# ppwwyyxx/OpenPano

Measured on NVIDIA H100. Metric: Mpixels/sec SIFT+match+blend, higher is better.
Workload: dtype f32

## Files before the change

openpano_b200/capi.py:

```python
from __future__ import annotations

import ctypes as C
import os
from pathlib import Path

import numpy as np

from ._abi import (PanoBaLink, PanoBaPair, PanoBlendGeom, PanoCylJob, PanoBlendImage, PanoMatches, PanoParams, PanoRansacPair, PanoSSPoint,
                   default_params)

LIB_PATH = Path(__file__).resolve().parent / "libpano_b200.so"

_fp = C.POINTER(C.c_float)
_dp = C.POINTER(C.c_double)
_ip = C.POINTER(C.c_int)
_vpp = C.POINTER(C.c_void_p)

SSPOINT_DTYPE = np.dtype([("x", "<i4"), ("y", "<i4"), ("real_x", "<f8"), ("real_y", "<f8"),
                          ("pyr_id", "<i4"), ("scale_id", "<i4"), ("dir", "<f4"),
                          ("scale_factor", "<f4")], align=True)


class PanoError(RuntimeError):
    def __init__(self, code, msg):
# ... 302 lines not shown
    def profile(self, on: bool):
        self._check(LIB.pano_profile_enable(self._h, 1 if on else 0))

    def profile_reset(self):
        self._check(LIB.pano_profile_reset(self._h))

    def profile_read(self):
        cap = 64
        names = C.create_string_buffer(cap * 64)
        launches = (C.c_int * cap)()
        ms = (C.c_double * cap)()
        n = LIB.pano_profile_read(self._h, cap, names, launches, ms)
        out = {}
        for i in range(min(n, cap)):
            nm = names.raw[i * 64:(i + 1) * 64].split(b"\0", 1)[0].decode()
            out[nm] = (launches[i], ms[i])
        return out

    def dev_alloc(self, nbytes):
        p = C.c_void_p()
        self._check(LIB.pano_dev_alloc(self._h, nbytes, C.byref(p)))
        return p.value

    def dev_free(self, ptr):
        LIB.pano_dev_free(self._h, C.c_void_p(ptr))

    def dev_upload(self, ptr, arr):
        arr = np.ascontiguousarray(arr)
        self._check(LIB.pano_dev_upload(self._h, C.c_void_p(ptr), arr.ctypes.data_as(C.c_void_p), arr.nbytes))

    def dev_download(self, arr, ptr):
        assert arr.flags.c_contiguous
        self._check(LIB.pano_dev_download(self._h, arr.ctypes.data_as(C.c_void_p), C.c_void_p(ptr), arr.nbytes))

    def dev_upload_async(self, d_ptr, h_ptr, nbytes):
        self._check(LIB.pano_dev_upload_async(self._h, C.c_void_p(d_ptr), C.c_void_p(h_ptr), nbytes))

    def dev_download_async(self, h_ptr, d_ptr, nbytes):
        self._check(LIB.pano_dev_download_async(self._h, C.c_void_p(h_ptr), C.c_void_p(d_ptr), nbytes))

    @staticmethod
    def host_alloc(nbytes):
        p = C.c_void_p()
        if LIB.pano_host_alloc(nbytes, C.byref(p)) != 0:
            raise PanoError(-1, "pano_host_alloc failed")
        return p.value

    @staticmethod
    def host_free(ptr):
        LIB.pano_host_free(C.c_void_p(ptr))

    def event_create(self):
        e = C.c_void_p()
        self._check(LIB.pano_event_create(self._h, C.byref(e)))
        return e

    def event_record(self, ev):
        self._check(LIB.pano_event_record(self._h, ev))

    def event_wait(self, ev):
        self._check(LIB.pano_event_wait(self._h, ev))

    @staticmethod
    def event_sync(ev):
        if LIB.pano_event_sync(ev) != 0:
            raise PanoError(-1, "pano_event_sync failed")

    @staticmethod
    def event_destroy(ev):
        LIB.pano_event_destroy(ev)

    def sift_detect_batch(self, imgs, params=None) -> FeatureSet:
        params = params or default_params()
        imgs = [np.ascontiguousarray(im, np.float32) for im in imgs]
        n = len(imgs)
        ptrs = (C.c_void_p * n)(*[im.ctypes.data for im in imgs])
        ws = (C.c_int * n)(*[im.shape[1] for im in imgs])
        hs = (C.c_int * n)(*[im.shape[0] for im in imgs])
        out = C.c_void_p()
        self._check(LIB.pano_sift_detect_batch(self._h, n, ptrs, ws, hs, C.byref(params), C.byref(out)))
        return FeatureSet(self, out)

    def sift_detect_batch_ptr(self, ptrs, ws, hs, params=None, device=False) -> FeatureSet:
        params = params or default_params()
        n = len(ptrs)
        cp = (C.c_void_p * n)(*ptrs)
        cw = (C.c_int * n)(*ws)
        ch = (C.c_int * n)(*hs)
        out = C.c_void_p()
        fn = LIB.pano_sift_detect_batch_dev if device else LIB.pano_sift_detect_batch
        self._check(fn(self._h, n, cp, cw, ch, C.byref(params), C.byref(out)))
        return FeatureSet(self, out)

    def sift_detect(self, img, params=None):
        fs = self.sift_detect_batch([img], params)
        try:
            return fs.download(0)
        finally:
            fs.free()

    def sift_trace(self, img, params=None) -> GpuSiftTrace:
        params = params or default_params()
        img = np.ascontiguousarray(img, np.float32)
        out = C.c_void_p()
        self._check(LIB.pano_sift_trace_run(self._h, _f(img), img.shape[1], img.shape[0], C.byref(params),
                                            C.byref(out)))
        return GpuSiftTrace(self, out)

    def featureset_upload(self, descs, coors=None) -> FeatureSet:
        descs = [np.ascontiguousarray(d, np.float32).reshape(-1, 128) for d in descs]
        n = len(descs)
        cnt = (C.c_int * n)(*[len(d) for d in descs])
        dp = (C.c_void_p * n)(*[d.ctypes.data for d in descs])
        cp = None
        if coors is not None:
            coors = [np.ascontiguousarray(c, np.float64).reshape(-1, 2) for c in coors]
            cp = (C.c_void_p * n)(*[c.ctypes.data for c in coors])
        out = C.c_void_p()
        self._check(LIB.pano_featureset_upload(self._h, n, cnt, dp, cp, C.byref(out)))
        return FeatureSet(self, out)

    def featureset_import_dev(self, counts, d_descs, d_coors=None) -> FeatureSet:
        n = len(counts)
        cnt = (C.c_int * n)(*counts)
        dp = (C.c_void_p * n)(*d_descs)
        cp = (C.c_void_p * n)(*d_coors) if d_coors is not None else None
        out = C.c_void_p()
        self._check(LIB.pano_featureset_import_dev(self._h, n, cnt, dp, cp, C.byref(out)))
        return FeatureSet(self, out)

    def blend_rows_dev(self, ptrs, shapes, items, geom, d_out_rows, out_w, out_h, row0, row1, bands=0, params=None):
        params = params or default_params()
        arr, g = self._blend_args(ptrs, shapes, items, geom)
        self._check(LIB.pano_blend_rows_dev(self._h, len(ptrs), arr, C.byref(g), bands, C.byref(params),
                                            C.c_void_p(d_out_rows), out_w, out_h, row0, row1))

    def match_pairs(self, fs: FeatureSet, pairs, params=None, shard=(0, 1)):
        params = params or default_params()
        pairs = np.ascontiguousarray(pairs, np.int32).reshape(-1, 2)
        m = PanoMatches()
        self._check(LIB.pano_match_pairs_shard(self._h, fs._h, len(pairs), _i(pairs), C.byref(params), int(shard[0]),
                                               int(shard[1]), C.byref(m)))
        n = m.n_pairs
        offs = np.ctypeslib.as_array(m.offset, shape=(n + 1,)).copy() if n else np.zeros(1, np.int32)
        total = int(offs[n]) if n else 0
        idx = (np.ctypeslib.as_array(m.idx, shape=(2 * total,)).reshape(-1, 2).copy() if total
               else np.zeros((0, 2), np.int32))
        LIB.pano_matches_free(C.byref(m))
        return [idx[offs[k]:offs[k + 1]] for k in range(n)]

    def match_pairs_dev(self, fs: FeatureSet, pairs, params=None, shard=(0, 1)) -> int:
        params = params or default_params()
        pairs = np.ascontiguousarray(pairs, np.int32).reshape(-1, 2)
        tot = C.c_int()
        self._check(LIB.pano_match_pairs_dev_shard(self._h, fs._h, len(pairs), _i(pairs), C.byref(params), int(shard[0]),
                                                   int(shard[1]), C.byref(tot)))
        return tot.value

    def match_bruteforce(self, a, b, params=None):
        params = params or default_params()
        a = np.ascontiguousarray(a, np.float32).reshape(-1, 128)
        b = np.ascontiguousarray(b, np.float32).reshape(-1, 128)
        pairs = np.zeros((max(1, min(len(a), len(b))), 2), np.int32)
        n = C.c_int()
        self._check(LIB.pano_match_bruteforce(self._h, _f(a), len(a), _f(b), len(b), C.byref(params),
                                              _i(pairs), C.byref(n)))
        return pairs[:n.value].copy()

    def ransac_score_pairs(self, pairs):
        n = len(pairs)
        arr = (PanoRansacPair * max(n, 1))()
# ... 22 lines not shown
            C.memmove(arr[k].m, np.ascontiguousarray(mats, np.float64).ctypes.data, 13 * 9 * 8)
            begin += nm
        pts_to = np.ascontiguousarray(pts_to, np.float64).reshape(-1, 2)
        assert len(pts_to) == begin
        rows = np.zeros((max(begin, 1), 24), np.float64) if want_rows else None
        jtj = np.full((6 * n_cam, 6 * n_cam), np.nan, np.float64)
        self._check(LIB.pano_ba_jacobian(self._h, n_cam, n, arr, _d(pts_to), _d(rows) if want_rows else None, _d(jtj)))
        return (rows[:begin] if want_rows else None), jtj

    def ba_session(self, n_cam, pairs, pts) -> BaSession:
        n = len(pairs)
        arr = (PanoBaLink * max(n, 1))()
        begin = 0
        for k, (f, t, nm) in enumerate(pairs):
            arr[k].from_, arr[k].to, arr[k].match_begin, arr[k].n_match = f, t, begin, nm
            begin += nm
        pts = np.ascontiguousarray(pts, np.float64).reshape(-1, 4)
        if len(pts) != begin:
            raise PanoError(-2, f"ba session: {len(pts)} coordinate rows for {begin} matches")
        h = C.c_void_p()
        self._check(LIB.pano_ba_session_create(self._h, n_cam, n, arr, _d(pts) if len(pts) else None, C.byref(h)))
        return BaSession(self, h, n_cam, n, begin)

    @staticmethod
    def cyl_warp_shape(w, h, h_factor=1.0, params=None):
        params = params or default_params()
        ow, oh, ox, oy = C.c_int(), C.c_int(), C.c_double(), C.c_double()
        rc = LIB.pano_cyl_warp_shape(w, h, h_factor, C.byref(params), C.byref(ow), C.byref(oh), C.byref(ox),
                                     C.byref(oy))
        if rc:
            raise PanoError(rc, "pano_cyl_warp_shape")
        return ow.value, oh.value, ox.value, oy.value

    def cyl_warp(self, img, kpts=None, h_factor=1.0, params=None):
        params = params or default_params()
        img = np.ascontiguousarray(img, np.float32)
        ow, oh, _, _ = self.cyl_warp_shape(img.shape[1], img.shape[0], h_factor, params)
        out = np.empty((oh, ow, 3), np.float32)
        k = np.ascontiguousarray(kpts if kpts is not None else np.zeros((0, 2)), np.float64).copy()
        self._check(LIB.pano_cyl_warp(self._h, _f(img), img.shape[1], img.shape[0], h_factor, C.byref(params),
                                      _f(out), ow, oh, _d(k), len(k)))
        return out, k

    def cyl_warp_batch_dev(self, src_ptrs, shapes, dst_ptrs, kpts=None, h_factor=1.0, params=None):
        params = params or default_params()
        n = len(src_ptrs)
        arr = (PanoCylJob * max(n, 1))()
        for k in range(n):
            h, w = shapes[k]
            ow, oh, _, _ = self.cyl_warp_shape(w, h, h_factor, params)
            arr[k].d_rgb_hwc, arr[k].w, arr[k].h = src_ptrs[k], w, h
            arr[k].d_out_hwc, arr[k].out_w, arr[k].out_h = dst_ptrs[k], ow, oh
            if kpts is not None and kpts[k] is not None and len(kpts[k]):
                assert kpts[k].dtype == np.float64 and kpts[k].flags["C_CONTIGUOUS"]
                arr[k].kpts_xy, arr[k].n_kpts = kpts[k].ctypes.data, len(kpts[k])
        self._check(LIB.pano_cyl_warp_batch_dev(self._h, n, arr, h_factor, C.byref(params)))

    @staticmethod
    def _blend_args(imgs_or_ptrs, shapes, items, geom):
        n = len(items)
        arr = (PanoBlendImage * n)()
        for k in range(n):
            arr[k].rgb_hwc = imgs_or_ptrs[k]
            arr[k].h, arr[k].w = shapes[k]
            arr[k].x0, arr[k].y0, arr[k].x1, arr[k].y1 = items[k][:4]
            for q in range(9):
                arr[k].homo_inv[q] = items[k][4][q]
        g = PanoBlendGeom(projection=geom["projection"], res_x=geom["res_x"], res_y=geom["res_y"],
                          proj_min_x=geom["proj_min_x"], proj_min_y=geom["proj_min_y"])
        return arr, g

    def blend(self, imgs, items, geom, bands=0, params=None):
        params = params or default_params()
        imgs = [np.ascontiguousarray(im, np.float32) for im in imgs]
        arr, g = self._blend_args([im.ctypes.data for im in imgs], [im.shape[:2] for im in imgs], items, geom)
        ow, oh = C.c_int(), C.c_int()
        LIB.pano_blend_target_size(len(imgs), arr, C.byref(ow), C.byref(oh))
        out = np.empty((oh.value, ow.value, 3), np.float32)
        self._check(LIB.pano_blend(self._h, len(imgs), arr, C.byref(g), bands, C.byref(params), _f(out),
                                   ow.value, oh.value))
        return out

    def blend_dev(self, ptrs, shapes, items, geom, d_out, out_w, out_h, bands=0, params=None):
        params = params or default_params()
        arr, g = self._blend_args(ptrs, shapes, items, geom)
        self._check(LIB.pano_blend_dev(self._h, len(ptrs), arr, C.byref(g), bands, C.byref(params),
                                       C.c_void_p(d_out), out_w, out_h))

    PLANET_SIZE = 1000

    def planet(self, img):
        img = np.ascontiguousarray(img, np.float32)
        if img.ndim != 3 or img.shape[2] != 3:
            raise PanoError(-2, f"planet: expected an H×W×3 image, got shape {img.shape}")
        out = np.empty((self.PLANET_SIZE, self.PLANET_SIZE, 3), np.float32)
        self._check(LIB.pano_planet(self._h, _f(img), img.shape[1], img.shape[0], _f(out)))
        return out

    def planet_dev(self, d_src, w, h, d_out):
        self._check(LIB.pano_planet_dev(self._h, C.c_void_p(d_src or 0), w, h, C.c_void_p(d_out or 0)))

    def rgb8_to_mat32f_batch_dev(self, d_pix, ws, hs, channels, d_out):
        n = len(d_pix)
        src = (C.c_void_p * n)(*d_pix)
        dst = (C.c_void_p * n)(*d_out)
        self._check(LIB.pano_rgb8_to_mat32f_batch_dev(self._h, n, src, (C.c_int * n)(*ws), (C.c_int * n)(*hs),
                                                      (C.c_int * n)(*channels), dst))

    def rgb8_to_mat32f_dev(self, d_pix, w, h, channels, d_out):
        self._check(LIB.pano_rgb8_to_mat32f_dev(self._h, C.c_void_p(d_pix), w, h, channels, C.c_void_p(d_out)))

    def crop_rect_dev(self, d_mat, w, h, d_rect):
        self._check(LIB.pano_crop_rect_dev(self._h, C.c_void_p(d_mat), w, h, C.c_void_p(d_rect)))

    def mat32f_to_rgb8_dev(self, d_mat, w, h, d_rect, d_out):
        self._check(LIB.pano_mat32f_to_rgb8_dev(self._h, C.c_void_p(d_mat), w, h, C.c_void_p(d_rect or 0),
                                                C.c_void_p(d_out)))

    def read_img_rgb8(self, pix):
        pix = np.ascontiguousarray(pix, np.uint8)
        h, w = pix.shape[:2]
        ch = 1 if pix.ndim == 2 else pix.shape[2]
        d_in = self.dev_alloc(max(pix.nbytes, 256))
        d_out = self.dev_alloc(h * w * 12)
        out = np.empty((h, w, 3), np.float32)
        try:
            self.dev_upload(d_in, pix)
            self.rgb8_to_mat32f_dev(d_in, w, h, ch, d_out)
            self.dev_download(out, d_out)
        finally:
            self.dev_free(d_in)
            self.dev_free(d_out)
        return out

    def crop_write_rgb8(self, mat, crop=True):
        mat = np.ascontiguousarray(mat, np.float32)
        h, w = mat.shape[:2]
        d_mat = self.dev_alloc(mat.nbytes)
        d_rect = self.dev_alloc(256)
        d_out = self.dev_alloc(max(h * w * 3, 256))
        rect = np.zeros(4, np.int32)
        out = np.empty(h * w * 3, np.uint8)
        try:
            self.dev_upload(d_mat, mat)
            if crop:
                self.crop_rect_dev(d_mat, w, h, d_rect)
            self.mat32f_to_rgb8_dev(d_mat, w, h, d_rect if crop else 0, d_out)
            self.dev_download(out, d_out)
            if crop:
                self.dev_download(rect, d_rect)
        finally:
            for p_ in (d_mat, d_rect, d_out):
                self.dev_free(p_)
        if not crop:
            return None, out.reshape(h, w, 3)
        cw, ch = int(rect[2]), int(rect[3])
        return rect, out[:cw * ch * 3].reshape(ch, cw, 3).copy()
```

openpano_b200/csrc/match.cu:

```cuda
#include "sift.cuh"
#include "match_tc.cuh"
#include <float.h>
#include <stdlib.h>
#include <string.h>
#include <algorithm>

__device__ __forceinline__ float exact_dist(const float* __restrict__ a, const float* __restrict__ b) {
  float l0 = 0.f, l1 = 0.f, l2 = 0.f, l3 = 0.f;
  const float4* pa = (const float4*)a;
  const float4* pb = (const float4*)b;
#pragma unroll 8
  for (int k = 0; k < 32; ++k) {
    float4 x = __ldg(pa + k), y = __ldg(pb + k);
    float d0 = x.x - y.x, d1 = x.y - y.y, d2 = x.z - y.z, d3 = x.w - y.w;
    l0 += d0 * d0; l1 += d1 * d1; l2 += d2 * d2; l3 += d3 * d3;
  }
  return (l0 + l1) + (l2 + l3);
}

__device__ __forceinline__ void top2_merge(float& mn, int& idx, float& sec, float m2, int i2, float s2) {
  if (m2 < mn || (m2 == mn && i2 < idx)) { sec = fminf(mn, s2); mn = m2; idx = i2; }
  else sec = fminf(sec, m2);
}

// ... 632 lines not shown
                (long long)pl.res_total, rs, pl.lazy ? 1 : 0, b.info);
  }
  if (pl.max_small > 0) {
    int block_cap = (int)std::min<size_t>(std::max<size_t>(pl.tc_tasks.size(), 1), 4096);
    if (const char* e = getenv("PANO_MATCH_BLOCK_CAP")) block_cap = std::max(1, std::min(block_cap, atoi(e)));
    const size_t grow = (size_t)block_cap * 128;
    TcFilter f;
    if ((rc = ctx_alloc(ctx, (void**)&b.list_rows, nres * sizeof(int))) ||
        (rc = ctx_alloc(ctx, (void**)&b.gtasks, (size_t)block_cap * sizeof(TcTask))) ||
        (rc = ctx_alloc(ctx, (void**)&b.gq, (size_t)block_cap * tc_block_bytes())) ||
        (rc = ctx_alloc(ctx, (void**)&b.g_meta, grow * sizeof(int2))) ||
        (rc = ctx_alloc(ctx, (void**)&b.g_thr, grow * sizeof(int))) ||
        (rc = ctx_alloc(ctx, (void**)&b.cand_cnt, grow * sizeof(int))) ||
        (rc = ctx_alloc(ctx, (void**)&b.cand, grow * TC_CAND_CAP * sizeof(int))))
      return rc;
    f.gq = b.gq; f.tasks = b.gtasks; f.gsides = b.gsides; f.list_rows = b.list_rows; f.approx = b.approx;
    f.g_meta = b.g_meta; f.g_thr = b.g_thr; f.cand_cnt = b.cand_cnt; f.cand = b.cand;
    TcFilter nf;
    int nom_cap = 0;
    if (pl.lazy) {
      nom_cap = (int)std::min<long long>(std::max<long long>(pl.large_blocks, 1), 8192);
      const size_t nrow = (size_t)nom_cap * 128;
      if ((rc = ctx_alloc(ctx, (void**)&b.list_unknown, nres * sizeof(int))) ||
          (rc = ctx_alloc(ctx, (void**)&b.ntasks, (size_t)nom_cap * sizeof(TcTask))) ||
          (rc = ctx_alloc(ctx, (void**)&b.nq, (size_t)nom_cap * tc_block_bytes())) ||
          (rc = ctx_alloc(ctx, (void**)&b.n_meta, nrow * sizeof(int2))) ||
          (rc = ctx_alloc(ctx, (void**)&b.n_approx, nrow * sizeof(TcTop2))))
        return rc;
      nf.gq = b.nq; nf.tasks = b.ntasks; nf.gsides = b.gsides; nf.list_rows = b.list_unknown; nf.approx = nullptr;
      nf.g_meta = b.n_meta; nf.g_thr = nullptr; nf.cand_cnt = nullptr; nf.cand = nullptr;
    }
    int* list_unknown = pl.lazy ? b.list_unknown : b.list_rows;
    const int eg = ctx->num_sms * 4;
    b.rounds = pl.lazy ? 3 : 2;
    for (int round = 0; round <= b.rounds; ++round) {
      int* side_cnt = b.counters + MC_HEAD + round * 2 * n_sides;
      int* fb_cnt = b.counters + MC_FB(round);
      int* n_blocks = b.counters + MC_BLK_FILTER(round);
      PANO_LAUNCH(ctx, "k_match_decide", k_match_decide, gd, 256, 0, b.pairs, b.sides, b.info, rs, round == 0 ? 1 : 0,
                  b.out, b.counters, b.list_rows, list_unknown, side_cnt, n_sides);
      if (round == b.rounds) break;
      if (pl.lazy) {
        int* nom_blocks = b.counters + MC_BLK_NOMINATE(round);
        PANO_LAUNCH(ctx, "k_gather_plan", k_gather_plan, ceil_div(n_sides, 128), 128, 0, b.gsides, n_sides,
                    side_cnt + n_sides, b.list_unknown, nom_cap, b.ntasks, nom_blocks, b.list, fb_cnt);
        nf.n_tasks = nom_blocks;
        if ((rc = tc_run_nominate(ctx, ops, &nf, nom_cap, b.n_approx))) return rc;
        PANO_LAUNCH(ctx, "k_refine_gathered", k_refine_gathered, nom_cap, 128, 0, fs->d_desc, ops->d_norms, ops->d_maxnorm,
                    b.sides, b.n_meta, b.n_approx, nom_blocks, rs, b.approx, b.info);
      }
      PANO_LAUNCH(ctx, "k_gather_plan", k_gather_plan, ceil_div(n_sides, 128), 128, 0, b.gsides, n_sides, side_cnt,
                  b.list_rows, block_cap, b.gtasks, n_blocks, b.list, fb_cnt);
      f.n_tasks = n_blocks;
      if ((rc = tc_run_filter(ctx, ops, &f, block_cap))) return rc;
      PANO_LAUNCH(ctx, "k_exact_cands", k_exact_cands, eg, 256, 0, fs->d_desc, b.sides, n_blocks, b.g_meta, b.cand_cnt,
                  b.cand, b.info, b.list, fb_cnt);
      PANO_LAUNCH(ctx, "k_exact_rows", k_exact_rows, eg, 256, 0, fs->d_desc, b.sides, b.list, fb_cnt, b.info);
    }
  }
  return PANO_OK;
}

static int ensure_tc_operands(pano_ctx* ctx, pano_featureset* fs, std::vector<TcImage>& imgs) {
  imgs.resize(fs->n_images);
  int blk = 0;
  for (int i = 0; i < fs->n_images; ++i) {
    TcImage& im = imgs[i];
    im.row0 = fs->base[i]; im.n = fs->h_count[i];
    im.n_pad = (im.n + 255) / 256 * 256;
    im.blk0 = blk;
    blk += im.n_pad / 128;
  }
  if (fs->tc_ready) return PANO_OK;
  int rc = tc_prepare(ctx, fs->d_desc, imgs, &fs->tc);
  if (rc) return rc;
  fs->tc_ready = true;
  return PANO_OK;
}

static int match_common(pano_ctx* ctx, pano_featureset* fs, int n_pairs, const int* ij, const pano_params* p,
                        int shard, int n_shards, MatchPlan& pl, MatchBuffers& b) {
  if (n_shards < 1 || shard < 0 || shard >= n_shards) return ctx_fail(ctx, PANO_ERR_INVALID, "shard %d of %d", shard, n_shards);
  pl.shard = shard; pl.n_shards = n_shards;
  int rc = featureset_sync_counts(fs);
  if (rc) return rc;
  const bool tensor = !use_exact_path();
  std::vector<TcImage> tcimgs;
  if (tensor && (rc = ensure_tc_operands(ctx, fs, tcimgs))) return rc;
  rc = build_plan(ctx, fs, n_pairs, ij, pl, tensor ? &tcimgs : nullptr);
  if (rc) return rc;
  return run_plan(ctx, fs, pl, p->match_reject_next_ratio, tensor, &fs->tc, b);
}

extern "C" {

int pano_match_pairs(pano_ctx* ctx, pano_featureset* fs, int n_pairs, const int* ij, const pano_params* p,
                     pano_matches* out) {
  return pano_match_pairs_shard(ctx, fs, n_pairs, ij, p, 0, 1, out);
}

int pano_match_pairs_shard(pano_ctx* ctx, pano_featureset* fs, int n_pairs, const int* ij, const pano_params* p,
                           int shard, int n_shards, pano_matches* out) {
  ctx_enter(ctx);
  if (!ctx || !fs || !out || n_pairs < 0 || (n_pairs && !ij) || !p) return PANO_ERR_INVALID;
  memset(out, 0, sizeof(*out));
  MatchPlan pl;
  MatchBuffers b;
  int rc = match_common(ctx, fs, n_pairs, ij, p, shard, n_shards, pl, b);
  if (rc) { free_buffers(ctx, b, false); return rc; }
  const size_t n_hdr = 3 + 2 * (size_t)n_pairs;
  const size_t cap = (size_t)std::max<long long>(pl.out_total, 1) * 2;
  int *d_hdr = nullptr, *d_dense = nullptr;
  if ((rc = ctx_alloc(ctx, (void**)&d_hdr, n_hdr * sizeof(int))) || (rc = ctx_alloc(ctx, (void**)&d_dense, cap * sizeof(int)))) {
    ctx_free(ctx, d_hdr); ctx_free(ctx, d_dense); free_buffers(ctx, b, false); return rc;
  }
  int* h_stage = (int*)ctx_ring(ctx, (n_hdr + cap) * sizeof(int));
  if (!h_stage) { ctx_free(ctx, d_hdr); ctx_free(ctx, d_dense); free_buffers(ctx, b, false); return ctx_fail(ctx, PANO_ERR_CUDA, "pinned ring allocation failed"); }
  auto finish = [&](int code) { ctx_free(ctx, d_hdr); ctx_free(ctx, d_dense); free_buffers(ctx, b, false); return code; };
  if ((rc = ctx_zero(ctx, d_hdr, 2 * sizeof(int)))) return finish(rc);
  if (n_pairs > 0) {
    ctx->launches += 4;
    k_match_count<<<n_pairs, 256, 0, ctx->stream>>>(b.pairs, b.out, n_pairs, d_hdr);
    k_match_offsets<<<1, 1024, 0, ctx->stream>>>(n_pairs, d_hdr);
    k_match_write<<<n_pairs, 256, 0, ctx->stream>>>(b.pairs, b.out, n_pairs, d_hdr, d_dense);
    k_match_download<<<std::max(1, std::min(ctx->num_sms, (int)(cap / 4096) + 1)), 256, 0, ctx->stream>>>(h_stage + n_hdr, d_dense, d_hdr);
    cudaError_t le = cudaGetLastError();
    if (le != cudaSuccess) return finish(ctx_cuda(ctx, le, "match result compaction"));
  }
  rc = ctx_store(ctx, h_stage, d_hdr, n_hdr * sizeof(int));
  cudaError_t e = ctx_spin_stream(ctx);
  if (rc) return finish(rc);
  if (e != cudaSuccess) return finish(ctx_cuda(ctx, e, "match download"));
  finish(0);
  if (n_pairs > 0 && h_stage[1] != 0) return ctx_fail(ctx, PANO_ERR_CUDA, "match: %d undecided rows (internal error)", h_stage[1]);
  const int total = n_pairs > 0 ? h_stage[0] : 0;
  out->n_pairs = n_pairs;
  out->count = (int*)calloc(std::max(n_pairs, 1), sizeof(int));
  out->offset = (int*)calloc(n_pairs + 1, sizeof(int));
  out->idx = (int*)calloc((size_t)std::max(total, 1) * 2, sizeof(int));
  if (n_pairs > 0) {
    memcpy(out->count, h_stage + 2, (size_t)n_pairs * sizeof(int));
    memcpy(out->offset, h_stage + 2 + n_pairs, (size_t)(n_pairs + 1) * sizeof(int));
    memcpy(out->idx, h_stage + n_hdr, (size_t)total * 2 * sizeof(int));
  }
  return PANO_OK;
}

void pano_matches_free(pano_matches* m) {
  if (!m) return;
  free(m->count); free(m->offset); free(m->idx);
  memset(m, 0, sizeof(*m));
}

int pano_match_pairs_dev(pano_ctx* ctx, pano_featureset* fs, int n_pairs, const int* ij, const pano_params* p,
                         int* total_matches) {
  return pano_match_pairs_dev_shard(ctx, fs, n_pairs, ij, p, 0, 1, total_matches);
}

int pano_match_pairs_dev_shard(pano_ctx* ctx, pano_featureset* fs, int n_pairs, const int* ij, const pano_params* p,
                               int shard, int n_shards, int* total_matches) {
  ctx_enter(ctx);
  if (!ctx || !fs || n_pairs < 0 || (n_pairs && !ij) || !p || !total_matches) return PANO_ERR_INVALID;
  MatchPlan pl;
  MatchBuffers b;
  int rc = match_common(ctx, fs, n_pairs, ij, p, shard, n_shards, pl, b);
  if (rc) { free_buffers(ctx, b, false); return rc; }
  int* h = (int*)ctx_ring(ctx, (size_t)std::max(b.n_counters, MC_HEAD) * sizeof(int));
// ... 49 lines not shown
```

openpano_b200/csrc/sift.cu:

```cuda
#include "sift.cuh"
#include "desc_interval.h"
#include <math.h>
#include <string.h>
#include <algorithm>
#include <cuda.h>

__device__ __forceinline__ void bilinear_coef(int d, float inv, int src_n, int* s, float* frac) {
  float r = ((float)d + 0.5f) * inv - 0.5f;
  int si = (int)floorf(r);
  r -= (float)si;
  if (si < 0) { si = 0; r = 0.f; }
  else if (si + 1 >= src_n) { si = src_n - 2; r = 1.f; }
  *s = si; *frac = r;
}

__global__ void k_working_resize(const ImgMeta* __restrict__ imgs, const OctMeta* __restrict__ octs, int n_oct,
                                 float* __restrict__ arena) {
  const ImgMeta im = imgs[blockIdx.z];
  int c = blockIdx.x * blockDim.x + threadIdx.x;
  int r = blockIdx.y * blockDim.y + threadIdx.y;
  if (c >= im.w0 || r >= im.h0) return;
  int sx, sy; float rx, ry;
  bilinear_coef(r, im.ifx, im.in_h, &sx, &rx);
  bilinear_coef(c, im.ify, im.in_w, &sy, &ry);
// ... 1370 lines not shown
    const void* srcs[4] = {wk->h_img.data(), wk->h_oct.data(), tilespan.data(), nullptr};
    size_t sizes[4] = {n * sizeof(ImgMeta), wk->h_oct.size() * sizeof(OctMeta), tilespan.size() * sizeof(int2),
                       (2 * n + 2) * sizeof(int)};
    SIFT_TRY(ctx_put_many(ctx, 4, dsts, srcs, sizes));
  }
  if (fast) {
    std::vector<TmaDesc> maps(n_om);
    const int R = gt.rmax;
    for (int k = 0; k < n_om; ++k) {
      const OctMeta& om = wk->h_oct[k];
      unsigned long long dims[2] = {(unsigned long long)om.w, (unsigned long long)om.h};
      unsigned long long strides[1] = {(unsigned long long)om.pitch * sizeof(float)};
      unsigned box[2] = {(unsigned)(BT_W + 2 * ((R + 3) & ~3)), (unsigned)(BT_H + 2 * R)};
      SIFT_TRY(ctx_tma_encode(ctx, &maps[k], wk->arena + om.gauss_off, 2, dims, strides, box));
    }
    SIFT_TRY(ctx_put(ctx, wk->d_maps, maps.data(), maps.size() * sizeof(TmaDesc)));
  }

#define SIFT_LAUNCH(name, kernel, grid, block, smem, ...)                                   \
  do {                                                                                      \
    ctx->launches++;                                                                        \
    if (ctx->profiling) ctx_prof_begin(ctx, name);                                          \
    kernel<<<(grid), (block), (smem), ctx->stream>>>(__VA_ARGS__);                          \
    if (ctx->profiling) ctx_prof_end(ctx);                                                  \
    SIFT_CUDA(cudaGetLastError());                                                          \
  } while (0)

  {
    dim3 b(32, 8), g(ceil_div(max_w0, 32), ceil_div(max_h0, 8), n);
    SIFT_LAUNCH("k_working_resize", k_working_resize, g, b, 0, wk->d_img, wk->d_oct, n_oct, wk->arena);
    if (n_oct > 1) {
      int max_w1 = 0, max_h1 = 0;
      for (int i = 0; i < n; ++i) {
        max_w1 = std::max(max_w1, wk->h_oct[(size_t)i * n_oct + 1].w);
        max_h1 = std::max(max_h1, wk->h_oct[(size_t)i * n_oct + 1].h);
      }
      dim3 g2(ceil_div(max_w1, 32), ceil_div(max_h1, 8), n * (n_oct - 1));
      SIFT_LAUNCH("k_octave_grey", k_octave_grey, g2, b, 0, wk->d_img, wk->d_oct, n_oct, wk->arena);
    }
  }
  {
    const ExtremaParams ep{n_scale, p->pre_color_thres, p->judge_extrema_diff_thres, cap, wk->cand_count, wk->cand_keys,
                           (int)seam_cap, wk->cand_count + n + 2, wk->seam_keys};
    const int R = gt.rmax;
    size_t smem = ((size_t)(BT_H + 2 * R) * (BT_W + 2 * R) + (size_t)BT_H * (BT_W + 2 * R)) * sizeof(float);
    if (smem > 200 * 1024) { sift_work_free(ctx, wk); return ctx_fail(ctx, PANO_ERR_INVALID, "sift: blur halo too large"); }
    if (fast) {
      const int GW = BT_W + 2 * ((R + 3) & ~3), GH = BT_H + 2 * R;
      const size_t gsz = ((size_t)GH * GW + 31) & ~(size_t)31;
      size_t smf = (2 * gsz + (size_t)BLUR_COLBUF_FLOATS(6) + (size_t)BT_H * (BT_W + 1) + EX_RING_FLOATS) * sizeof(float);
      SIFT_CUDA(cudaFuncSetAttribute(k_blur_extrema, cudaFuncAttributeMaxDynamicSharedMemorySize, (int)smf));
      const int grid = std::min(wk->n_tiles, ctx->num_sms * 3);
      SIFT_LAUNCH("k_blur_extrema", k_blur_extrema, grid, BT_THREADS, smf, wk->d_oct, wk->d_tilespan, n_om, wk->n_tiles,
                  wk->d_maps, wk->arena, gt, ep);
      SIFT_LAUNCH("k_extrema_seams", k_extrema_seams, dim3(8, n), 256, 0, wk->d_oct, n_oct, wk->arena, ep);
    } else {
      if (smem > 48 * 1024)
        SIFT_CUDA(cudaFuncSetAttribute(k_blur_dog, cudaFuncAttributeMaxDynamicSharedMemorySize, (int)smem));
      SIFT_LAUNCH("k_blur_dog_generic", k_blur_dog, wk->n_tiles, BT_THREADS, smem, wk->d_oct, wk->d_tilespan, n_om, wk->arena, gt);
      SIFT_LAUNCH("k_extrema_scan", k_extrema_scan, wk->n_tiles, EXS_THREADS, 0, wk->d_oct, wk->d_tilespan, n_om,
                  wk->arena, ep);
    }
  }
  {
    dim3 g(8, n);
    SIFT_LAUNCH("k_rank_sort", k_rank_sort, g, 256, 0, wk->cand_count, wk->cand_keys, wk->sorted_keys, cap);
    RefineParams rp{n_scale, p->calc_offset_depth, p->offset_thres, p->contrast_thres, p->edge_ratio,
                    p->gauss_sigma, p->scale_factor};
    dim3 g4(16, n);
    SIFT_LAUNCH("k_refine", k_refine, g4, 128, 0, wk->d_oct, wk->arena, n_oct, wk->cand_count, wk->sorted_keys, rp, cap,
                wk->refined, wk->kp_valid);
    const char* ori_env = getenv("PANO_ORI_V1");
    const bool ori_v1 = ori_env && atoi(ori_env) != 0;
    if (ori_v1)
      SIFT_LAUNCH("k_orientation", k_orientation_v1, ctx->num_sms * 8, ORI_WARPS * 32, 0, wk->d_oct, wk->arena, n_oct, n, cap,
                  wk->cand_count, wk->refined, wk->kp_valid, p->ori_radius, p->ori_hist_smooth_count, wk->npeaks, wk->dirs,
                  wk->cand_count + n + 1);
    else
      SIFT_LAUNCH("k_orientation", k_orientation, ctx->num_sms * 8, ORI_WARPS * 32, 0, wk->d_oct, wk->arena, n_oct, n, cap,
                  wk->cand_count, wk->refined, wk->kp_valid, p->ori_radius, p->ori_hist_smooth_count, wk->npeaks, wk->dirs,
                  wk->cand_count + n + 1);
    SIFT_LAUNCH("k_expand_scan", k_expand_scan, n, SCAN_THREADS, 0, wk->cand_count, wk->kp_valid, wk->npeaks,
                wk->dirs, cap, fs->d_count, wk->n_refined, wk->desc_cand, wk->desc_dir);
    DescParams dp{p->desc_hist_scale_factor, p->desc_int_factor};
    const char* desc_env = getenv("PANO_DESC_V1");
    const bool desc_v1 = desc_env && atoi(desc_env) != 0;
    int grid = ctx->num_sms * DESC_CTAS_PER_SM;
    if (desc_v1) {
      const size_t dsm = sizeof(DescWarpSmem) * DESC_WARPS;
      SIFT_CUDA(cudaFuncSetAttribute(k_descriptor_v1, cudaFuncAttributeMaxDynamicSharedMemorySize, (int)dsm));
      SIFT_LAUNCH("k_descriptor", k_descriptor_v1, grid, DESC_THREADS, dsm, wk->d_oct, wk->d_img, wk->arena, n_oct, n, cap,
                  wk->refined, fs->d_count, wk->desc_cand, wk->desc_dir, dp, fs->d_desc, fs->d_coor, wk->cand_count + n);
    } else {
      const size_t dsm = sizeof(DescQuadSmem) * DESC_WARPS;
      SIFT_CUDA(cudaFuncSetAttribute(k_descriptor, cudaFuncAttributeMaxDynamicSharedMemorySize, (int)dsm));
      grid = ctx->num_sms * DESC_MIN_CTAS;
      SIFT_LAUNCH("k_descriptor", k_descriptor, grid, DESC_THREADS, dsm, wk->d_oct, wk->d_img, wk->arena, n_oct, n, cap,
                  wk->refined, fs->d_count, wk->desc_cand, wk->desc_dir, dp, fs->d_desc, fs->d_coor, wk->cand_count + n);
    }
  }
  wk->n_desc = fs->d_count;

  if (!fs->h_count_pinned) {
    fs->h_count_pinned = (int*)ctx_small_pinned_get(ctx, (size_t)2 * n * sizeof(int) + 16, &fs->h_count_cap);
    if (!fs->h_count_pinned) { sift_work_free(ctx, wk); return ctx_fail(ctx, PANO_ERR_CUDA, "pinned allocation failed"); }
  }
  {
    void* dsts[2] = {fs->h_count_pinned, fs->h_count_pinned + n};
    const void* srcs[2] = {fs->d_count, wk->cand_count};
    size_t sizes[2] = {n * sizeof(int), n * sizeof(int)};
    SIFT_TRY(ctx_store_many(ctx, 2, dsts, srcs, sizes));
  }
  SIFT_CUDA(ctx_signal(ctx, &fs->counts_token));
  fs->counts_pending = true;
  fs->counts_on_host = false;

  if (keep) *keep = wk;
  else sift_work_free(ctx, wk);
  return PANO_OK;
}

int featureset_sync_counts(pano_featureset* fs) {
  SlowCall sc("featureset_sync_counts");
  if (fs->error) return fs->error;
  if (fs->counts_on_host) return PANO_OK;
  pano_ctx* ctx = fs->ctx;
  while (fs->counts_pending) {
    cudaError_t e = ctx_wait_signal(ctx, fs->counts_token);
    if (e != cudaSuccess) return fs->error = ctx_cuda(ctx, e, "feature count read-back");
    fs->counts_pending = false;
    const int n = fs->n_images;
    int worst = 0;
    for (int i = 0; i < n; ++i) worst = std::max(worst, std::max(fs->h_count_pinned[i], fs->h_count_pinned[n + i]));
    if (worst <= fs->cap) {
      fs->h_count.assign(fs->h_count_pinned, fs->h_count_pinned + n);
      break;
    }
    int cap = fs->cap;
    while (cap < worst && cap < SIFT_CAP_MAX) cap *= 2;
    if (cap < worst || fs->src.empty())
      return fs->error = ctx_fail(ctx, PANO_ERR_CAPACITY, "sift: %d list entries in one image exceed the capacity %d", worst, fs->cap);
    ctx_free(ctx, fs->d_desc); ctx_free(ctx, fs->d_coor); ctx_free(ctx, fs->d_count);
    fs->d_desc = nullptr; fs->d_coor = nullptr; fs->d_real = nullptr; fs->d_count = nullptr;
    ctx->sift_cap = cap;
    const std::vector<const float*> src = fs->src;
    int rc = sift_run_batch(ctx, n, src.data(), fs->src_w.data(), fs->src_h.data(), &fs->src_params, fs, nullptr, cap);
    if (rc) return fs->error = rc;
  }
  if (fs->owned_block) { ctx_free(ctx, fs->owned_block); fs->owned_block = nullptr; }
  fs->counts_on_host = true;
  return PANO_OK;
}
```

openpano_b200/csrc/sift.cuh:

```cuda
#pragma once
#include "common.cuh"
#include "match_tc.cuh"

#define SIFT_MAX_OCT 8
#define SIFT_MAX_LEVELS 8
#define SIFT_MAX_TAPS 32
#define SIFT_CAP_DEFAULT 8192
#define SIFT_CAP_MAX (1 << 20)
#define SIFT_MAX_PEAKS 18

struct ImgMeta {
  const float* src;
  int in_w, in_h;
  int w0, h0;
  float ifx, ify;
  long long work_off;
};

struct OctMeta {
  int img, oct;
  int w, h;
  int pitch;
  float ifx, ify;
  long long gauss_off;
  long long plane;
};

struct GaussTable {
  int nlev;
  int rmax;
  int center[SIFT_MAX_LEVELS];
  float taps[SIFT_MAX_LEVELS][SIFT_MAX_TAPS];
};

struct SiftWork {
  int n_img = 0, n_oct = 0, n_scale = 0;
  std::vector<ImgMeta> h_img;
  std::vector<OctMeta> h_oct;
  float* arena = nullptr;
  size_t arena_floats = 0;
  ImgMeta* d_img = nullptr;
  OctMeta* d_oct = nullptr;
  int2* d_tilespan = nullptr;
  TmaDesc* d_maps = nullptr;
  int n_tiles = 0;
  int cap = SIFT_CAP_DEFAULT;
  int* cand_count = nullptr;
  uint32_t* cand_keys = nullptr;
  uint32_t* seam_keys = nullptr;
  uint32_t* sorted_keys = nullptr;
  pano_sspoint* refined = nullptr;
  unsigned char* kp_valid = nullptr;
  int* npeaks = nullptr;
  float* dirs = nullptr;
  int* n_desc = nullptr;
  int* n_refined = nullptr;
  int* desc_cand = nullptr;
  float* desc_dir = nullptr;
};

struct pano_featureset {
  pano_ctx* ctx = nullptr;
  int n_images = 0;
  float* d_desc = nullptr;
  double* d_coor = nullptr;
  double* d_real = nullptr;
  int* d_count = nullptr;
  std::vector<long long> base;
  std::vector<int> h_count;
  bool counts_on_host = false;
  cudaEvent_t counts_ready = nullptr;
  unsigned counts_token = 0;
  bool counts_pending = false;
  int* h_count_pinned = nullptr;
  size_t h_count_cap = 0;
  TcOperands tc;
  bool tc_ready = false;
  int error = 0;
  int cap = 0;
  std::vector<const float*> src;
  std::vector<int> src_w, src_h;
  pano_params src_params;
  float* owned_block = nullptr;
};

int sift_run_batch(pano_ctx* ctx, int n, const float* const* d_src, const int* w, const int* h,
                   const pano_params* p, pano_featureset* fs, SiftWork** keep, int cap);
void sift_work_free(pano_ctx* ctx, SiftWork* wk);
int featureset_sync_counts(pano_featureset* fs);
```

openpano_b200/stitcher.py:

```python
from __future__ import annotations

import numpy as np

from ._abi import default_params
from .capi import Engine


from .synth import all_pairs, ordered_pairs


class Stitcher:
    def __init__(self, engine: Engine, params=None, overlap_blend: bool = True):
        self.eng = engine
        self.params = params or default_params()
        self._aux = None
        self._overlap = overlap_blend
        self._ev_in = self._ev_blend = None
        self._d_imgs = None
        self._d_out = None
        self._shapes = None
        self._offs = None
        self._out_shape = None

    def _ensure(self, shapes, out_wh):
        if self._shapes != shapes:
            self.release_images()
            offs, total = [], 0
            for (h, w) in shapes:
                offs.append(total)
                total += (h * w * 3 * 4 + 255) // 256 * 256
            self._d_imgs = self.eng.dev_alloc(max(total, 256))
            self._shapes, self._offs = list(shapes), offs
        if self._out_shape != out_wh:
            if self._d_out:
                self.eng.dev_free(self._d_out)
            self._d_out = self.eng.dev_alloc(max(out_wh[0] * out_wh[1] * 3 * 4, 256))
            self._out_shape = out_wh

    def release_images(self):
        if self._d_imgs:
            self.eng.dev_free(self._d_imgs)
            self._d_imgs = None
            self._shapes = None

    def close(self):
        self.release_images()
        if self._d_out:
            self.eng.dev_free(self._d_out)
            self._d_out = None
            self._out_shape = None
        if self._aux is not None:
            self._aux.sync()
            Engine.event_destroy(self._ev_in)
            Engine.event_destroy(self._ev_blend)
            self._aux.close()
            self._aux = None

    def _aux_engine(self):
        if self._aux is None:
            self._aux = Engine(self.eng.device)
            self._ev_in = self.eng.event_create()
            self._ev_blend = self._aux.event_create()
        return self._aux

    def image_ptrs(self):
        return [self._d_imgs + o for o in self._offs]

    def upload(self, host_ptrs, shapes, out_wh):
        self._ensure(list(shapes), tuple(out_wh))
        for p, o, (h, w) in zip(host_ptrs, self._offs, shapes):
            self.eng.dev_upload_async(self._d_imgs + o, p, h * w * 3 * 4)

    def run_device(self, pairs, items, geom, bands=0, want_matches=False):
        shapes = self._shapes
        ptrs = self.image_ptrs()
        if self._overlap:
            aux = self._aux_engine()
            self.eng.event_record(self._ev_in)
            aux.event_wait(self._ev_in)
            aux.blend_dev(ptrs, shapes, items, geom, self._d_out, self._out_shape[0], self._out_shape[1], bands, self.params)
            aux.event_record(self._ev_blend)
        fs = self.eng.sift_detect_batch_ptr(ptrs, [s[1] for s in shapes], [s[0] for s in shapes], self.params,
                                            device=True)
        if want_matches:
            m = self.eng.match_pairs(fs, pairs, self.params)
        else:
            m = self.eng.match_pairs_dev(fs, pairs, self.params)
        if self._overlap:
            self.eng.event_wait(self._ev_blend)
        else:
            self.eng.blend_dev(ptrs, shapes, items, geom, self._d_out, self._out_shape[0], self._out_shape[1], bands,
                               self.params)
        return fs, m

    def build(self, host_ptrs, shapes, pairs, items, geom, out_host_ptr, bands=0):
        out_w = max(it[2] for it in items)
        out_h = max(it[3] for it in items)
        self.upload(host_ptrs, shapes, (out_w, out_h))
        fs, matches = self.run_device(pairs, items, geom, bands, want_matches=True)
        self.eng.dev_download_async(out_host_ptr, self._d_out, out_w * out_h * 3 * 4)
        self.eng.sync()
        fs.free()
        return matches

    def build_numpy(self, imgs, pairs, items, geom, bands=0):
        imgs = [np.ascontiguousarray(im, np.float32) for im in imgs]
        out_w = max(it[2] for it in items)
        out_h = max(it[3] for it in items)
        out = np.empty((out_h, out_w, 3), np.float32)
        m = self.build([im.ctypes.data for im in imgs], [im.shape[:2] for im in imgs], pairs, items, geom,
                       out.ctypes.data, bands)
        return m, out


class PipelinedStitcher:

    def __init__(self, device: int, params=None, depth: int = 2, rgb8: bool = False, crop: bool = True):
        self.params = params or default_params()
        self.up = Engine(device)
        self.cmp = Engine(device)
        self.dn = Engine(device)
        self.depth = depth
        self.rgb8 = rgb8
        self.crop = crop
        self.slots = [dict(imgs=None, out=None, shapes=None, offs=None, out_wh=None, pix=None, pix_offs=None, out8=None,
                           ev_up=self.up.event_create(), ev_cmp=self.cmp.event_create(),
                           ev_dn=self.dn.event_create(), busy=False) for _ in range(depth)]
        self._next = 0

    def _ensure(self, s, shapes, out_wh):
        realloc = False
        if s["shapes"] != shapes:
            realloc = True
            if s["imgs"]:
                self.cmp.dev_free(s["imgs"])
            offs, total = [], 0
            for (h, w) in shapes:
                offs.append(total)
                total += (h * w * 3 * 4 + 255) // 256 * 256
            s["imgs"] = self.cmp.dev_alloc(max(total, 256))
            s["shapes"], s["offs"] = list(shapes), offs
            if self.rgb8:
                if s["pix"]:
                    self.cmp.dev_free(s["pix"])
                poffs, ptotal = [], 0
                for (h, w) in shapes:
                    poffs.append(ptotal)
                    ptotal += (h * w * 3 + 255) // 256 * 256
                s["pix"] = self.cmp.dev_alloc(max(ptotal, 256))
                s["pix_offs"] = poffs
        if s["out_wh"] != out_wh:
            if s["out"]:
                self.cmp.dev_free(s["out"])
            s["out"] = self.cmp.dev_alloc(max(out_wh[0] * out_wh[1] * 3 * 4, 256))
            if self.rgb8:
                if s["out8"]:
                    self.cmp.dev_free(s["out8"])
                s["out8"] = self.cmp.dev_alloc(self.out_bytes(out_wh))
            s["out_wh"] = tuple(out_wh)
            realloc = True
        if realloc:
            self.cmp.sync()

    RGB8_HEADER = 256

    def out_bytes(self, out_wh) -> int:
        if self.rgb8:
            return self.RGB8_HEADER + out_wh[0] * out_wh[1] * 3
        return out_wh[0] * out_wh[1] * 3 * 4

    def in_bytes(self, shapes) -> int:
        return sum(h * w * 3 * (1 if self.rgb8 else 4) for (h, w) in shapes)

    def stage(self, host_ptrs, shapes, out_wh) -> int:
        k = self._next
# ... 144 lines not shown
```

Baseline: 10890.

## Read back feature counts before descriptor kernels and cache ctypes argument arrays

The feature-count device-to-host copy and its completion signal are now issued right after the expand-scan, before the descriptor kernels, so the host can learn the counts and start planning matches while descriptors are still being computed. A separate descriptor-completion token is waited on only when the matcher runs on a different context. The stitcher also caches the ctypes argument arrays for SIFT and blend between calls, which removes per-call Python marshalling. The cache relies on deepcopied key comparisons, and the split signalling adds synchronisation complexity across contexts.

After: 11030, median of 6. No clear change (+1.3%).

```diff
diff --git a/openpano_b200/capi.py b/openpano_b200/capi.py
--- a/openpano_b200/capi.py
+++ b/openpano_b200/capi.py
@@ -408,11 +408,16 @@
         return FeatureSet(self, out)
 
     def sift_detect_batch_ptr(self, ptrs, ws, hs, params=None, device=False) -> FeatureSet:
-        params = params or default_params()
+        return self.sift_detect_batch_args(self.sift_args(ptrs, ws, hs), params, device)
+
+    @staticmethod
+    def sift_args(ptrs, ws, hs):
         n = len(ptrs)
-        cp = (C.c_void_p * n)(*ptrs)
-        cw = (C.c_int * n)(*ws)
-        ch = (C.c_int * n)(*hs)
+        return (n, (C.c_void_p * n)(*ptrs), (C.c_int * n)(*ws), (C.c_int * n)(*hs))
+
+    def sift_detect_batch_args(self, args, params=None, device=False) -> FeatureSet:
+        params = params or default_params()
+        n, cp, cw, ch = args
         out = C.c_void_p()
         fn = LIB.pano_sift_detect_batch_dev if device else LIB.pano_sift_detect_batch
         self._check(fn(self._h, n, cp, cw, ch, C.byref(params), C.byref(out)))
@@ -601,9 +606,13 @@
         return out
 
     def blend_dev(self, ptrs, shapes, items, geom, d_out, out_w, out_h, bands=0, params=None):
-        params = params or default_params()
-        arr, g = self._blend_args(ptrs, shapes, items, geom)
-        self._check(LIB.pano_blend_dev(self._h, len(ptrs), arr, C.byref(g), bands, C.byref(params),
+        self.blend_dev_args((len(ptrs),) + self._blend_args(ptrs, shapes, items, geom), d_out, out_w, out_h, bands,
+                            params)
+
+    def blend_dev_args(self, args, d_out, out_w, out_h, bands=0, params=None):
+        params = params or default_params()
+        n, arr, g = args
+        self._check(LIB.pano_blend_dev(self._h, n, arr, C.byref(g), bands, C.byref(params),
                                        C.c_void_p(d_out), out_w, out_h))
 
     PLANET_SIZE = 1000
diff --git a/openpano_b200/csrc/match.cu b/openpano_b200/csrc/match.cu
--- a/openpano_b200/csrc/match.cu
+++ b/openpano_b200/csrc/match.cu
@@ -738,7 +738,7 @@
                         int shard, int n_shards, MatchPlan& pl, MatchBuffers& b) {
   if (n_shards < 1 || shard < 0 || shard >= n_shards) return ctx_fail(ctx, PANO_ERR_INVALID, "shard %d of %d", shard, n_shards);
   pl.shard = shard; pl.n_shards = n_shards;
-  int rc = featureset_sync_counts(fs);
+  int rc = featureset_sync_counts(fs, ctx != fs->ctx);
   if (rc) return rc;
   const bool tensor = !use_exact_path();
   std::vector<TcImage> tcimgs;
diff --git a/openpano_b200/csrc/sift.cu b/openpano_b200/csrc/sift.cu
--- a/openpano_b200/csrc/sift.cu
+++ b/openpano_b200/csrc/sift.cu
@@ -1476,6 +1476,19 @@
                   wk->cand_count + n + 1);
     SIFT_LAUNCH("k_expand_scan", k_expand_scan, n, SCAN_THREADS, 0, wk->cand_count, wk->kp_valid, wk->npeaks,
                 wk->dirs, cap, fs->d_count, wk->n_refined, wk->desc_cand, wk->desc_dir);
+    if (!fs->h_count_pinned) {
+      fs->h_count_pinned = (int*)ctx_small_pinned_get(ctx, (size_t)2 * n * sizeof(int) + 16, &fs->h_count_cap);
+      if (!fs->h_count_pinned) { sift_work_free(ctx, wk); return ctx_fail(ctx, PANO_ERR_CUDA, "pinned allocation failed"); }
+    }
+    {
+      void* dsts[2] = {fs->h_count_pinned, fs->h_count_pinned + n};
+      const void* srcs[2] = {fs->d_count, wk->cand_count};
+      size_t sizes[2] = {n * sizeof(int), n * sizeof(int)};
+      SIFT_TRY(ctx_store_many(ctx, 2, dsts, srcs, sizes));
+    }
+    SIFT_CUDA(ctx_signal(ctx, &fs->counts_token));
+    fs->counts_pending = true;
+    fs->counts_on_host = false;
     DescParams dp{p->desc_hist_scale_factor, p->desc_int_factor};
     const char* desc_env = getenv("PANO_DESC_V1");
     const bool desc_v1 = desc_env && atoi(desc_env) != 0;
@@ -1494,31 +1507,26 @@
     }
   }
   wk->n_desc = fs->d_count;
-
-  if (!fs->h_count_pinned) {
-    fs->h_count_pinned = (int*)ctx_small_pinned_get(ctx, (size_t)2 * n * sizeof(int) + 16, &fs->h_count_cap);
-    if (!fs->h_count_pinned) { sift_work_free(ctx, wk); return ctx_fail(ctx, PANO_ERR_CUDA, "pinned allocation failed"); }
-  }
-  {
-    void* dsts[2] = {fs->h_count_pinned, fs->h_count_pinned + n};
-    const void* srcs[2] = {fs->d_count, wk->cand_count};
-    size_t sizes[2] = {n * sizeof(int), n * sizeof(int)};
-    SIFT_TRY(ctx_store_many(ctx, 2, dsts, srcs, sizes));
-  }
-  SIFT_CUDA(ctx_signal(ctx, &fs->counts_token));
-  fs->counts_pending = true;
-  fs->counts_on_host = false;
+  SIFT_CUDA(ctx_signal(ctx, &fs->desc_token));
+  fs->desc_pending = true;
 
   if (keep) *keep = wk;
   else sift_work_free(ctx, wk);
   return PANO_OK;
 }
 
-int featureset_sync_counts(pano_featureset* fs) {
+int featureset_sync_counts(pano_featureset* fs, bool need_desc) {
   SlowCall sc("featureset_sync_counts");
   if (fs->error) return fs->error;
-  if (fs->counts_on_host) return PANO_OK;
   pano_ctx* ctx = fs->ctx;
+  if (fs->counts_on_host) {
+    if (need_desc && fs->desc_pending) {
+      cudaError_t e = ctx_wait_signal(ctx, fs->desc_token);
+      if (e != cudaSuccess) return fs->error = ctx_cuda(ctx, e, "descriptor completion");
+      fs->desc_pending = false;
+    }
+    return PANO_OK;
+  }
   while (fs->counts_pending) {
     cudaError_t e = ctx_wait_signal(ctx, fs->counts_token);
     if (e != cudaSuccess) return fs->error = ctx_cuda(ctx, e, "feature count read-back");
@@ -1543,5 +1551,5 @@
   }
   if (fs->owned_block) { ctx_free(ctx, fs->owned_block); fs->owned_block = nullptr; }
   fs->counts_on_host = true;
-  return PANO_OK;
-}
+  return featureset_sync_counts(fs, need_desc);
+}
diff --git a/openpano_b200/csrc/sift.cuh b/openpano_b200/csrc/sift.cuh
--- a/openpano_b200/csrc/sift.cuh
+++ b/openpano_b200/csrc/sift.cuh
@@ -72,6 +72,8 @@
   cudaEvent_t counts_ready = nullptr;
   unsigned counts_token = 0;
   bool counts_pending = false;
+  unsigned desc_token = 0;
+  bool desc_pending = false;
   int* h_count_pinned = nullptr;
   size_t h_count_cap = 0;
   TcOperands tc;
@@ -87,4 +89,4 @@
 int sift_run_batch(pano_ctx* ctx, int n, const float* const* d_src, const int* w, const int* h,
                    const pano_params* p, pano_featureset* fs, SiftWork** keep, int cap);
 void sift_work_free(pano_ctx* ctx, SiftWork* wk);
-int featureset_sync_counts(pano_featureset* fs);
+int featureset_sync_counts(pano_featureset* fs, bool need_desc = true);
diff --git a/openpano_b200/stitcher.py b/openpano_b200/stitcher.py
--- a/openpano_b200/stitcher.py
+++ b/openpano_b200/stitcher.py
@@ -1,4 +1,6 @@
 from __future__ import annotations
+
+import copy
 
 import numpy as np
 
@@ -21,6 +23,19 @@
         self._shapes = None
         self._offs = None
         self._out_shape = None
+        self._sift_key = self._sift_args = None
+        self._blend_key = self._blend_args = None
+
+    def _cached_args(self, ptrs, shapes, items, geom):
+        key = (ptrs, shapes)
+        if key != self._sift_key:
+            self._sift_args = Engine.sift_args(ptrs, [s[1] for s in shapes], [s[0] for s in shapes])
+            self._sift_key = copy.deepcopy(key)
+        key = (ptrs, shapes, items, geom)
+        if key != self._blend_key:
+            self._blend_args = (len(ptrs),) + Engine._blend_args(ptrs, shapes, items, geom)
+            self._blend_key = copy.deepcopy(key)
+        return self._sift_args, self._blend_args
 
     def _ensure(self, shapes, out_wh):
         if self._shapes != shapes:
@@ -74,14 +89,14 @@
     def run_device(self, pairs, items, geom, bands=0, want_matches=False):
         shapes = self._shapes
         ptrs = self.image_ptrs()
+        sift_args, blend_args = self._cached_args(ptrs, shapes, items, geom)
         if self._overlap:
             aux = self._aux_engine()
             self.eng.event_record(self._ev_in)
             aux.event_wait(self._ev_in)
-            aux.blend_dev(ptrs, shapes, items, geom, self._d_out, self._out_shape[0], self._out_shape[1], bands, self.params)
+            aux.blend_dev_args(blend_args, self._d_out, self._out_shape[0], self._out_shape[1], bands, self.params)
             aux.event_record(self._ev_blend)
-        fs = self.eng.sift_detect_batch_ptr(ptrs, [s[1] for s in shapes], [s[0] for s in shapes], self.params,
-                                            device=True)
+        fs = self.eng.sift_detect_batch_args(sift_args, self.params, device=True)
         if want_matches:
             m = self.eng.match_pairs(fs, pairs, self.params)
         else:
@@ -89,8 +104,7 @@
         if self._overlap:
             self.eng.event_wait(self._ev_blend)
         else:
-            self.eng.blend_dev(ptrs, shapes, items, geom, self._d_out, self._out_shape[0], self._out_shape[1], bands,
-                               self.params)
+            self.eng.blend_dev_args(blend_args, self._d_out, self._out_shape[0], self._out_shape[1], bands, self.params)
         return fs, m
 
     def build(self, host_ptrs, shapes, pairs, items, geom, out_host_ptr, bands=0):
```
